# QZ1-boy/FCVSR

Hardware: AMD Instinct MI355X
Metric: SR frames/sec (7-frame window, 4x 180x320->720x1280) + PSNR vs ref (higher is better)
Workload: dtype bf16

## Files before the change

fcvsr_amd/engine.py:

```python
from __future__ import annotations

import ctypes as C
import math
import weakref
from collections import OrderedDict
from typing import Dict, List, Optional, Tuple

import numpy as np
import torch

from . import hip
from .hip import ACT_LEAKY, ACT_NONE, ACT_PRELU, ACT_RELU, check, lib, ptr, stream_ptr, view


_MASKS: Dict[Tuple[int, int, int], torch.Tensor] = {}


def band_masks_half(Q: int, H: int, W: int) -> torch.Tensor:
    key = (Q, H, W)
    if key not in _MASKS:
        n = 1024
        step = math.sqrt((n / 2) ** 2 + (n / 2) ** 2) / Q
        d2 = (np.arange(-(n // 2), n - n // 2, 1) ** 2).astype(np.float64)
        r2 = np.power(np.sqrt(d2[:, None] + d2[None, :]), 2)
# ... 140 lines not shown
    def _mask(self, Q, H, W, dev):
        key = (Q, H, W, str(dev))
        if key not in self._dev_masks:
            self._dev_masks[key] = band_masks_half(Q, H, W).to(dev)
        return self._dev_masks[key]

    def _conv(self, name, srcs, dst, *, stride=1, act=ACT_NONE, slope=0.0, slope_t=None, res=(), res_scale=(),
              ps=False, freq=False, direct=False, force_f16=False, rows=None, cols=None):
        self._convg(name, [dict(srcs=srcs, dst=dst, res=res, ps=ps)], stride=stride, act=act, slope=slope,
                    slope_t=slope_t, res_scale=res_scale, ps=ps, freq=freq, direct=direct, force_f16=force_f16, rows=rows,
                    cols=cols)
        return dst

    def _convg(self, name, groups, *, stride=1, act=ACT_NONE, slope=0.0, slope_t=None, res_scale=(), ps=False,
               freq=False, direct=False, force_f16=False, gc_wmask=None, rows=None, cols=None):
        ksz = self._par[name + ".weight"].shape[-1]
        any16 = any(t.dtype != torch.float32 for g in groups for t in list(g["srcs"]) + [g["dst"]])
        elig = self.precision != "f32" and not direct and hip.mfma_eligible(ksz, stride, groups)
        if any16 and not elig:
            raise RuntimeError(f"{name}: 16-bit activations require the MFMA path (ineligible shape/alignment)")
        if elig:
            dt = torch.bfloat16 if (self.precision == "bf16" or freq) else torch.float16
            if force_f16:
                dt = torch.float16
            w, b, cout, _ = self._weights(name, dt, ps, rows, cols)
            hip.conv2d_mfma(groups, w, ksz, cout, hip.BF16 if dt == torch.bfloat16 else hip.F16, stride=stride, bias=b, act=act,
                            slope=slope, slope_t=slope_t, res_scale=res_scale, pixel_shuffle=ps, gc_wmask=gc_wmask,
                            name=name)
            return True
        w, b, cout, _ = self._weights(name, "direct", False, rows, cols)
        wm = bm = None
        if (ksz in (1, 3) and stride == 1 and not direct and all(len(g["srcs"]) == 1 and g["srcs"][0].shape[3] % 32 == 0
                                                                  for g in groups) and (not ps or cout % 16 == 0)):
            wm, bm = self._weights(name, "f32mfma", ps, rows, cols)[:2]
        for g in groups:
            hip.conv2d(g["srcs"], w, ksz, cout, g["dst"], bias=b, stride=stride, act=act, slope=slope, slope_t=slope_t,
                       res=g.get("res", ()), res_scale=res_scale, pixel_shuffle=ps, name=name, w_f32mfma=wm, bias_f32mfma=bm)
        return False

    def _tap(self, name, t_nhwc):
        if self.taps is not None:
            self.taps[name] = t_nhwc.float().permute(0, 3, 1, 2).contiguous().clone()

    @staticmethod
    def _new(dev, *shape, dtype=torch.float32):
        return torch.empty(*shape, device=dev, dtype=dtype)

    def _channel_sum(self, t):
        B, H, W, Cc = t.shape
        nblk = (H * W + 255) // 256
        out = self._new(t.device, B, Cc)
        scratch = self._new(t.device, B * nblk * Cc)
        v = view(t)
        check(lib().fcvsr_channel_sum(C.byref(v), B, H, W, out.data_ptr(), scratch.data_ptr(), scratch.numel(),
                                      stream_ptr()), "fcvsr_channel_sum")
        return out

    def _ca_gate(self, sums, inv_hw, prefix, Bn, c):
        par = self._par
        w1, w2 = par[prefix + ".conv_du.0.weight"], par[prefix + ".conv_du.2.weight"]
        gate = self._new(sums.device, Bn, c)
        check(lib().fcvsr_ca_gate(sums.data_ptr(), inv_hw, w1.data_ptr(), w2.data_ptr(), Bn, c, w1.shape[0],
                                  gate.data_ptr(), stream_ptr()), "fcvsr_ca_gate")
        return gate

    def _mgaa(self, x1, x2, x3, tag):
        m = self._model()
        n, A = m.n_feats, m.ACNum
        dev = x1.device
        B, H, W, _ = x1.shape
        Wf = W // 2 + 1
        L = lib()
        st = stream_ptr()
        par = self._par

        spec = self._new(dev, 3, B, H, Wf, 2 * n)
        fs = 2 * n
        for i, xi in enumerate((x1, x2, x3)):
            v = view(xi)
            check(L.fcvsr_rfft2(C.byref(v), B, H, W, n, spec[i].data_ptr(), fs, 0, n, st), "fcvsr_rfft2")
        x1f, x2f, x3f = spec[0], spec[1], spec[2]

        fdt = self._adt(freq=True)
        off = self._new(dev, 2 * B, H, Wf, 2 * n, dtype=fdt)
        fused = fdt != torch.float32 and n == 64
        if fused:
            ws = [self._weights(f"MGAA.convfuse.{i}", torch.bfloat16)[0] for i in (0, 2, 4)]
            P2 = C.c_void_p * 2
            check(L.fcvsr_freq_mlp3(P2(x1f.data_ptr(), x3f.data_ptr()), P2(x2f.data_ptr(), x2f.data_ptr()), 2, fs,
                                    B * H * Wf, ws[0].data_ptr(), ws[1].data_ptr(), ws[2].data_ptr(),
                                    P2(off[:B].data_ptr(), off[B:].data_ptr()), 2 * n, st), "fcvsr_freq_mlp3")
        else:
            t0 = self._new(dev, 2 * B, H, Wf, 2 * n, dtype=fdt)
            t1 = self._new(dev, 2 * B, H, Wf, 2 * n, dtype=fdt)
            dirs = list(enumerate((x1f, x3f)))
            self._convg("MGAA.convfuse.0", [dict(srcs=[xa, x2f], dst=t0[d * B:(d + 1) * B]) for d, xa in dirs],
                        act=ACT_RELU, freq=True)
            self._convg("MGAA.convfuse.2", [dict(srcs=[t0], dst=t1)], act=ACT_RELU, freq=True)
            self._convg("MGAA.convfuse.4", [dict(srcs=[t1[d * B:(d + 1) * B]], dst=off[d * B:(d + 1) * B], res=[xa, x2f])
                                            for d, xa in dirs], res_scale=[1.0, -1.0], freq=True)
        sim = self._new(dev, B, H, Wf, 4)
        off4 = self._new(dev, 2 * B, H, Wf, 4)
        if fused:
            check(L.fcvsr_freq_head(x2f.data_ptr(), hip.F32, fs, B * H * Wf,
                                    self._weights("MGAA.convcrt.0", torch.bfloat16)[0].data_ptr(), None,
                                    self._weights("MGAA.convcrt.2", torch.bfloat16)[0].data_ptr(), sim.data_ptr(), st),
                  "fcvsr_freq_head(convcrt)")
        else:
            s0 = self._new(dev, B, H, Wf, n, dtype=fdt)
            self._conv("MGAA.convcrt.0", [x2f], s0, act=ACT_RELU, freq=True)
            self._conv("MGAA.convcrt.2", [s0], sim, freq=True)

        if fdt == torch.float32:
            c0 = self._new(dev, 2 * B, H, Wf, n, dtype=fdt)
            c1 = self._new(dev, 2 * B, H, Wf, n, dtype=fdt)
            corr = self._new(dev, B, H, Wf, 84)
            cv = view(corr)
            check(L.fcvsr_corr_lookup(x1f.data_ptr(), x2f.data_ptr(), fs, B, H, Wf, 2 * n, 4, Wf, C.byref(cv), st),
                  "fcvsr_corr_lookup")
            for d in range(2):
                self._conv("MGAA.convcorr.0", [off[d * B:(d + 1) * B], corr], c0[d * B:(d + 1) * B], act=ACT_RELU, freq=True)
            self._conv("MGAA.convcorr.2", [c0], c1, act=ACT_RELU, freq=True)
            self._conv("MGAA.convcorr.4", [c1], off4, freq=True)
        else:
            if fused:
                check(L.fcvsr_freq_head(off.data_ptr(), hip.BF16, 2 * n, 2 * B * H * Wf,
                                        self._weights("MGAA.convcorr.0", torch.bfloat16, cols=(0, 2 * n))[0].data_ptr(),
                                        self._weights("MGAA.convcorr.2", torch.bfloat16)[0].data_ptr(),
                                        self._weights("MGAA.convcorr.4", torch.bfloat16)[0].data_ptr(), off4.data_ptr(), st),
                      "fcvsr_freq_head(convcorr)")
            else:
                c0 = self._new(dev, 2 * B, H, Wf, n, dtype=fdt)
                c1 = self._new(dev, 2 * B, H, Wf, n, dtype=fdt)
                self._conv("MGAA.convcorr.0", [off], c0, act=ACT_RELU, freq=True, cols=(0, 2 * n))
            xs = min(Wf, 8)
            corr = self._new(dev, B, H, xs, 84)
            cv = view(corr)
            check(L.fcvsr_corr_lookup(x1f.data_ptr(), x2f.data_ptr(), fs, B, H, Wf, 2 * n, 4, xs, C.byref(cv), st),
                  "fcvsr_corr_lookup")
            off_s = off[:, :, :xs].to(torch.float32, memory_format=torch.contiguous_format)
            c0_s = self._new(dev, 2 * B, H, xs, n, dtype=fdt)
            for d in range(2):
                self._conv("MGAA.convcorr.0", [off_s[d * B:(d + 1) * B], corr], c0_s[d * B:(d + 1) * B], act=ACT_RELU,
                           freq=True)
            if fused:
                c1_s = self._new(dev, 2 * B, H, xs, n, dtype=fdt)
                off4_s = self._new(dev, 2 * B, H, xs, 4)
                self._conv("MGAA.convcorr.2", [c0_s], c1_s, act=ACT_RELU, freq=True)
                self._conv("MGAA.convcorr.4", [c1_s], off4_s, freq=True)
                off4[:, :, :xs].copy_(off4_s)
            else:
                c0[:, :, :xs].copy_(c0_s)
                self._conv("MGAA.convcorr.2", [c0], c1, act=ACT_RELU, freq=True)
                self._conv("MGAA.convcorr.4", [c1], off4, freq=True)

        ospec = self._new(dev, B, H, Wf, 8 * A)
        u = self._new(dev, 2 * B, H, Wf, 4)
        ntile = ((H + 15) // 16) * ((Wf + 15) // 16)
        partial = self._new(dev, 2 * B * ntile * 4)
        for i in range(A):
            pre = f"MGAA.MConvB.{i}"
            w1 = self._weights(pre + ".conv1", "direct")[0]
            w2 = self._weights(pre + ".conv2", "direct")[0]
            check(L.fcvsr_convblk(off4.data_ptr(), w1.data_ptr(), w2.data_ptr(), par[pre + ".relu.weight"].data_ptr(),
                                  par[pre + ".conv1.weight"].shape[-1], par[pre + ".CA.conv_du.0.weight"].data_ptr(),
                                  par[pre + ".CA.conv_du.2.weight"].data_ptr(), sim.data_ptr(), B, 2, H, Wf, u.data_ptr(),
                                  partial.data_ptr(), partial.numel(), ospec.data_ptr(), 8 * A, 0, 4 * A, A, i, st),
                  "fcvsr_convblk")
        offsets = self._new(dev, B, H, W, 4 * A)
        ov = view(offsets)
        check(L.fcvsr_irfft2(ospec.data_ptr(), 8 * A, 4 * A, 0, B, H, W, 4 * A, None, None, C.byref(ov), st),
              "fcvsr_irfft2")

        kp = self._new(dev, B, H, W, n, dtype=self._adt())
        k0 = self._new(dev, B, H, W, n, dtype=self._adt())
        fused_iac = n % 32 == 0
        self._conv("MGAA.conv_KP", [x2], kp)
        self._conv("MGAA.F.0", [kp], k0)
        fold_f1 = fused_iac and n == 64 and self.precision != "f32" and self._model().fold_f1
        if not fold_f1:
            K = self._new(dev, B, H, W, A * 3 * n, dtype=self._adt() if fused_iac else torch.float32)
            self._conv("MGAA.F.1", [k0], K)

        fdt_act = x1.dtype
        al = self._new(dev, B, H, W, 2 * n, dtype=fdt_act)
        ping = [self._new(dev, B, H, W, n, dtype=fdt_act), self._new(dev, B, H, W, n, dtype=fdt_act)]
        if not fused_iac:
            if fdt_act != torch.float32:
                raise RuntimeError("16-bit activations need the fused IAC kernel (n_features % 32 == 0)")
            s = self._new(dev, B, H, W, n)
            vbuf = self._new(dev, B, H, W, n)
        if fused_iac and n % 64 == 0:
            ping2 = [self._new(dev, B, H, W, n, dtype=fdt_act), self._new(dev, B, H, W, n, dtype=fdt_act)]
            V2 = hip.View * 2
            cur = [x1, x3]
            fins = V2(view(x1), view(x3))
            if fold_f1:
                wk, bk, _, _ = self._weights("MGAA.F.1", self._adt())
                k0_v = view(k0)
            for i in range(A):
                if not fold_f1:
                    k_v = view(K[..., i * 3 * n:(i + 1) * 3 * n])
                if i == A - 1:
                    dsts = [al[..., :n], al[..., n:]]
                else:
                    dsts = [ping[i % 2], ping2[i % 2]]
                prevs = V2(view(cur[0]), view(cur[1]))
                offs = V2(view(offsets[..., 2 * i:2 * i + 2]), view(offsets[..., 2 * (A + i):2 * (A + i) + 2]))
                dv2 = V2(view(dsts[0]), view(dsts[1]))
                if fold_f1:
                    check(L.fcvsr_iac_step2_fused(prevs, offs, C.byref(k0_v), wk.data_ptr() + i * 3 * n * 64 * 2,
                                                  bk.data_ptr() + i * 3 * n * 4, fins, 0.1, B, H, W, dv2, st),
                          "fcvsr_iac_step2_fused")
                else:
                    check(L.fcvsr_iac_step2(prevs, offs, C.byref(k_v), fins, 0.1, B, H, W, dv2, st), "fcvsr_iac_step2")
                cur = dsts
        else:
            for d, fin in enumerate((x1, x3)):
                cur = fin
                fv = view(fin)
                for i in range(A):
                    g = d * A + i
                    o_v = view(offsets[..., 2 * g:2 * g + 2])
# ... 381 lines not shown
```

fcvsr_amd/hip.py:

```python
from __future__ import annotations

import ctypes as C
import os
from typing import Optional, Sequence

import torch

_HERE = os.path.dirname(os.path.abspath(__file__))
LIB_PATH = os.path.join(_HERE, "lib", "libfcvsr_hip.so")

F32, BF16, F16 = 0, 1, 2
ACT_NONE, ACT_RELU, ACT_LEAKY, ACT_PRELU = 0, 1, 2, 3
_DT = {torch.float32: F32, torch.bfloat16: BF16, torch.float16: F16}


class View(C.Structure):
    _fields_ = [("ptr", C.c_void_p), ("sb", C.c_int64), ("sy", C.c_int64), ("sx", C.c_int64), ("sc", C.c_int64),
                ("c", C.c_int32), ("dtype", C.c_int32)]


class GcFinishLevel(C.Structure):
    _fields_ = [("partial", C.c_void_p), ("add", C.c_void_p), ("nparts", C.c_int32)]


class GcPartialLevel(C.Structure):
    _fields_ = [("r", C.c_void_p), ("partial", C.c_void_p), ("B", C.c_int32), ("H", C.c_int32), ("W", C.c_int32)]


class GcApplyLevel(C.Structure):
    _fields_ = [("r", C.c_void_p), ("add", C.c_void_p), ("z", C.c_void_p), ("out", C.c_void_p), ("pool", C.c_void_p),
                ("B", C.c_int32), ("H", C.c_int32), ("W", C.c_int32)]


class XscaleLevel(C.Structure):
    _fields_ = [("x", C.c_void_p), ("r", C.c_void_p), ("dn", C.c_void_p), ("up", C.c_void_p), ("out", C.c_void_p),
                ("r_scale", C.c_float), ("dn_pooled", C.c_int32), ("B", C.c_int32), ("H", C.c_int32), ("W", C.c_int32)]


class RcbTailArgs(C.Structure):
    _fields_ = [("x", C.c_void_p * 3), ("r", C.c_void_p * 3), ("z", C.c_void_p * 3), ("add", C.c_void_p * 3),
                ("out", C.c_void_p * 3), ("r1", C.c_void_p), ("u1", C.c_void_p), ("u2", C.c_void_p), ("w_up", C.c_void_p),
                ("b_up", C.c_void_p), ("w_dn", C.c_void_p), ("b_dn", C.c_void_p), ("B", C.c_int32), ("H", C.c_int32),
                ("W", C.c_int32)]


class ConvDesc(C.Structure):
    _fields_ = [("n_src", C.c_int32), ("src", View * 3), ("B", C.c_int32), ("H", C.c_int32), ("W", C.c_int32),
                ("kh", C.c_int32), ("kw", C.c_int32), ("stride", C.c_int32), ("pad", C.c_int32),
                ("cout", C.c_int32), ("weight", C.c_void_p), ("cout_pad", C.c_int32), ("bias", C.c_void_p),
                ("act", C.c_int32), ("slope", C.c_float), ("slope_ptr", C.c_void_p), ("n_res", C.c_int32),
                ("res", View * 2), ("res_scale", C.c_float * 2), ("dst", View), ("pixel_shuffle", C.c_int32),
                ("gc_wmask", C.c_void_p), ("gc_partial", C.c_void_p)]


PROFILE = None
COMPUTE_DTYPE = "f32"
DOMINANT_KERNEL = "conv_direct_kernel"


class HipError(RuntimeError):
    pass


_lib: Optional[C.CDLL] = None

_VP, _I, _I64, _F = C.c_void_p, C.c_int, C.c_int64, C.c_float
_PV = C.POINTER(View)
SIGNATURES = {
    "fcvsr_last_error": [],
    "fcvsr_last_conv_kernel": [],
    "fcvsr_conv2d_wgrad_scratch_elems": [C.c_int] * 7,
    "fcvsr_conv2d_wgrad": [C.c_void_p, C.c_void_p, C.c_int, C.c_int, C.c_int, C.c_int, C.c_int, C.c_int, C.c_int, C.c_void_p, C.c_void_p,
                           C.c_longlong, C.c_int, C.c_void_p],
    "fcvsr_conv2d_wgrad_mfma_eligible": [C.c_int] * 6,
    "fcvsr_conv2d_wgrad_mfma_scratch_elems": [C.c_int] * 7,
    "fcvsr_conv2d_wgrad_mfma": [C.c_void_p, C.c_void_p, C.c_int, C.c_int, C.c_int, C.c_int, C.c_int, C.c_int, C.c_int, C.c_void_p, C.c_void_p,
                                C.c_void_p, C.c_longlong, C.c_int, C.c_int, C.c_void_p],
    "fcvsr_abi_version": [],
    "fcvsr_device_count": [],
    "fcvsr_conv2d": [C.POINTER(ConvDesc), _VP],
    "fcvsr_conv2d_f32mfma": [C.POINTER(ConvDesc), _VP],
    "fcvsr_conv2d_f32mfma_eligible": [C.POINTER(ConvDesc)],
    "fcvsr_conv2d_mfma": [C.POINTER(ConvDesc), _I, _I, _VP],
    "fcvsr_rfft2": [_PV, _I, _I, _I, _I, _VP, _I64, _I, _I, _VP],
    "fcvsr_irfft2": [_VP, _I64, _I, _I, _I, _I, _I, _I, _VP, _VP, _PV, _VP],
    "fcvsr_irfft2_bands": [_VP, _I64, _I, _I, _I, _I, _I, _I, _VP, _I, _VP, _PV, _VP],
    "fcvsr_corr_lookup": [_VP, _VP, _I64, _I, _I, _I, _I, _I, _I, _PV, _VP],
    "fcvsr_channel_sum": [_PV, _I, _I, _I, _VP, _VP, _I64, _VP],
    "fcvsr_ca_gate": [_VP, _F, _VP, _VP, _I, _I, _I, _VP, _VP],
    "fcvsr_convblk_tail": [_VP, _VP, _VP, _I, _I, _I, _I, _VP, _I64, _I, _I, _I, _I, _VP],
    "fcvsr_convblk": [_VP, _VP, _VP, _VP, _I, _VP, _VP, _VP, _I, _I, _I, _I, _VP, _VP, _I64, _VP, _I64, _I, _I, _I, _I, _VP],
    "fcvsr_warp": [_PV, _PV, _I, _I, _I, _PV, _VP],
    "fcvsr_sac_v": [_PV, _PV, _I, _I, _I, _PV, _VP],
    "fcvsr_sac_h": [_PV, _PV, _PV, _F, _I, _I, _I, _PV, _VP],
    "fcvsr_iac_step": [_PV, _PV, _PV, _PV, _F, _I, _I, _I, _PV, _VP],
    "fcvsr_feat_extract": [_PV, _I, _I, _I, _VP, _VP, _I, _VP, _VP, _VP, _I, _VP],
    "fcvsr_freq_head": [_VP, _I, _I64, _I64, _VP, _VP, _VP, _VP, _VP],
    "fcvsr_freq_mlp3": [_VP, _VP, _I, _I64, _I64, _VP, _VP, _VP, _VP, _I64, _VP],
    "fcvsr_iac_step2": [_PV, _PV, _PV, _PV, _F, _I, _I, _I, _PV, _VP],
    "fcvsr_iac_step2_fused": [_PV, _PV, _PV, _VP, _VP, _PV, _F, _I, _I, _I, _PV, _VP],
    "fcvsr_divenh": [_I, _I, _VP, _VP, _VP, _VP, _VP, _VP, _F, _VP, _VP, _VP, _VP, _I64, _I, _I, _I, _I, _VP],
    "fcvsr_divenh_apply_next": [_I, _VP, _VP, _VP, _VP, _VP, _VP, _F, _VP, _VP, _VP, _VP, _VP, _VP, _VP, _I64, _I, _I, _I, _I, _VP],
    "fcvsr_scale_add": [_VP, _VP, _VP, _I, _VP, _I, _I, _I, _I, _I, _VP],
    "fcvsr_gc_context": [_VP, _VP, _VP, _VP, _I, _I, _I, _I, _VP, _VP, _I64, _VP],
    "fcvsr_gc_finish": [_VP, _I, _VP, _VP, _I, _I, _VP, _VP],
    "fcvsr_gc_apply": [_VP, _VP, _VP, _VP, _I, _F, _I, _I, _I, _I, _VP],
    "fcvsr_xscale": [_VP, _VP, _F, _VP, _VP, _VP, _I, _I, _I, _I, _I, _VP],
    "fcvsr_gc_finish_levels": [C.POINTER(GcFinishLevel), _I, _VP, _VP, _I, _I, _VP],
    "fcvsr_gc_partial_levels": [C.POINTER(GcPartialLevel), _I, _I, _VP, _I, _VP],
    "fcvsr_gc_apply_levels": [C.POINTER(GcApplyLevel), _I, _I, _I, _F, _I, _VP],
    "fcvsr_xscale_levels": [C.POINTER(XscaleLevel), _I, _I, _I, _VP],
    "fcvsr_rcb_level0": [_VP, _VP, _VP, _VP, _VP, _VP, _VP, _F, _F, _I, _I, _I, _I, _I, _VP],
    "fcvsr_rcb_tail": [C.POINTER(RcbTailArgs), _F, _I, _I, _VP],
    "fcvsr_pixel_shuffle": [_VP, _VP, _I, _I, _I, _I, _VP],
    "fcvsr_bilinear_up4": [_PV, _I, _I, _I, _PV, _VP],
    "fcvsr_tail_fused": [_PV, _VP, _VP, _VP, _VP, _VP, _I, _I, _I, _PV, _VP],
    "fcvsr_conv_last": [_PV, _VP, _VP, _I, _I, _I, _I, _PV, _VP],
    "fcvsr_pack_weight_mfma": [_VP, _I, _I, _I, _I, _VP, _I, _I, _I, _I, _VP],
    "fcvsr_pack_weights_multi_block_elems": [],
    "fcvsr_pack_weights_mfma_multi": [_VP, _I, _I, _I, _VP],
    "fcvsr_act_bwd": [_VP, _VP, _VP, _F, C.c_longlong, _VP],
    "fcvsr_colsum_scratch_elems": [C.c_longlong, _I],
    "fcvsr_colsum": [_VP, C.c_longlong, _I, _VP, _VP, C.c_longlong, _I, _VP],
    "fcvsr_iac_bwd_sac": [_VP, _VP, _VP, _VP, _PV, _F, _I, _I, _I, _I, _VP, _I, _VP, _PV, _I, _VP],
    "fcvsr_iac_bwd_warp": [_VP, _PV, _VP, _PV, _I, _I, _I, _I, _VP, _VP, _VP],
    "fcvsr_prelu_fwd": [_VP, _VP, _VP, C.c_longlong, _VP],
    "fcvsr_prelu_bwd": [_VP, _VP, _VP, _VP, _VP, _VP, C.c_longlong, _VP],
    "fcvsr_wgrad_cout1_scratch_elems": [_I, _I, _I],
    "fcvsr_wgrad_cout1": [_VP, _VP, _I, _I, _I, _I, _VP, _VP, C.c_longlong, _I, _VP],
    "fcvsr_conv2d_wgrad_mfma_groups_scratch_elems": [_VP, _VP, _VP, _I, _I, _I, _I, _I],
    "fcvsr_conv2d_wgrad_mfma_groups": [_VP, _VP, _VP, _VP, _VP, _I, _I, _I, _I, _VP, _VP, _VP, C.c_longlong, _I, _I, _VP],
    "fcvsr_up2_adjoint": [_VP, _VP, _I, _I, _I, _I, _VP],
    "fcvsr_pool2_adjoint": [_VP, _VP, _I, _I, _I, _I, _VP],
    "fcvsr_rcbt_nblk": [_I],
    "fcvsr_rcbt_stat_elems": [],
    "fcvsr_rcbt_forward": [_VP, _VP, _VP, _VP, _VP, _F, _I, _I, _I, _VP, _VP, _VP, C.c_longlong, _VP],
    "fcvsr_rcbt_backward": [_VP, _VP, _VP, _VP, _VP, _VP, _F, _I, _I, _I, _VP, _VP, _VP, _VP, _VP, C.c_longlong, _I, _VP],
    "fcvsr_divenh_band_nblk": [_I],
    "fcvsr_divenh_band_stat_elems": [_I],
    "fcvsr_divenh_band_forward": [_VP, _VP, _VP, _VP, _VP, _VP, _VP, _I, _I, _I, _VP, _VP, _VP, _VP, C.c_longlong, _VP],
    "fcvsr_divenh_band_backward": [_VP, _VP, _VP, _VP, _VP, _VP, _VP, _VP, _VP, _VP, _I, _I, _I, _VP, _VP, _VP, _VP, _VP, _VP, _VP, _VP,
                                   C.c_longlong, _I, _VP],
    "fcvsr_corr_lookup_bwd": [_VP, _VP, _I64, _I, _I, _I, _I, _I, _I, _PV, _VP, _VP, _VP],
    "fcvsr_frame_metrics_scratch_bytes": [_I] * 6,
    "fcvsr_frame_metrics": [_VP, C.POINTER(C.c_int64), _I, _VP, C.POINTER(C.c_int64), _I, _I, _I, _I, _I, _I,
                            C.POINTER(C.c_double), _VP, _VP, C.c_longlong, _VP],
}
_RESTYPES = {"fcvsr_last_error": C.c_char_p, "fcvsr_last_conv_kernel": C.c_char_p, "fcvsr_conv2d_wgrad_scratch_elems": C.c_longlong,
             "fcvsr_conv2d_wgrad_mfma_scratch_elems": C.c_longlong, "fcvsr_colsum_scratch_elems": C.c_longlong,
             "fcvsr_wgrad_cout1_scratch_elems": C.c_longlong, "fcvsr_conv2d_wgrad_mfma_groups_scratch_elems": C.c_longlong,
             "fcvsr_frame_metrics_scratch_bytes": C.c_longlong}


def lib() -> C.CDLL:
    global _lib
    if _lib is None:
        if not os.path.exists(LIB_PATH):
            raise HipError(f"{LIB_PATH} not found: run `python -m fcvsr_amd.build` (hipcc, gfx950). "
                           "fcvsr_amd has no CPU fallback.")
        l = C.CDLL(LIB_PATH)
        for name, args in SIGNATURES.items():
            fn = getattr(l, name, None)
            if fn is None:
                continue
            fn.argtypes = args
            fn.restype = _RESTYPES.get(name, C.c_int)
        _lib = l
    return _lib


def check(rc: int, what: str) -> None:
    if rc != 0:
        msg = lib().fcvsr_last_error()
        raise HipError(f"{what} failed (rc={rc}): {msg.decode() if msg else ''}")


def stream_ptr() -> int:
    return torch.cuda.current_stream().cuda_stream


def view(t: torch.Tensor) -> View:
# ... 164 lines not shown
```

include/fcvsr_hip.h:

```cpp
#ifndef FCVSR_HIP_H
#define FCVSR_HIP_H

#include <stdint.h>

#ifdef __cplusplus
extern "C" {
#endif

#define FCVSR_ABI_VERSION 2

enum { FCVSR_E_ARG = -1, FCVSR_E_UNSUPPORTED = -2, FCVSR_E_NOGPU = -3 };
enum { FCVSR_F32 = 0, FCVSR_BF16 = 1, FCVSR_F16 = 2 };
enum { FCVSR_ACT_NONE = 0, FCVSR_ACT_RELU = 1, FCVSR_ACT_LEAKY = 2, FCVSR_ACT_PRELU = 3 };

typedef struct fcvsr_view {
  void*   ptr;
  int64_t sb, sy, sx, sc;
  int32_t c;
  int32_t dtype;
} fcvsr_view;

typedef struct fcvsr_conv_desc {
  int32_t     n_src;
  fcvsr_view  src[3];
// ... 37 lines not shown
                           int transposed, void* stream);
int fcvsr_pack_weights_multi_block_elems(void);
int fcvsr_pack_weights_mfma_multi(const long long* tab, int n_items, int total_blocks, int dtype, void* stream);
int fcvsr_act_bwd(const float* g, const float* y, float* out, float slope, long long n, void* stream);
long long fcvsr_colsum_scratch_elems(long long npix, int C);
int fcvsr_colsum(const float* x, long long npix, int C, float* out, float* scratch, long long scratch_elems, int accumulate, void* stream);
int fcvsr_rcbt_nblk(int HW);
int fcvsr_rcbt_stat_elems(void);
int fcvsr_rcbt_forward(const float* r, const float* z, const float* wmask, const float* w1, const float* w2, float slope, int B, int HW,
                       int C, float* out, float* stats, float* scratch, long long scratch_elems, void* stream);
int fcvsr_rcbt_backward(const float* r, const float* g, const float* wmask, const float* w1, const float* w2, const float* stats,
                        float slope, int B, int HW, int C, float* gr, float* dwmask, float* dw1, float* dw2, float* scratch,
                        long long scratch_elems, int accumulate , void* stream);

int fcvsr_divenh_band_nblk(int HW);
int fcvsr_divenh_band_stat_elems(int C);
int fcvsr_divenh_band_forward(const float* f, const float* sf, const float* so, const float* a, const float* b, const float* w1,
                              const float* w2, int B, int HW, int C, float* sf_out, float* so_out, float* stats, float* scratch,
                              long long scratch_elems, void* stream);
int fcvsr_divenh_band_backward(const float* f, const float* sf, const float* so, const float* a, const float* b, const float* w1,
                               const float* w2, const float* stats, const float* gsf, const float* gso, int B, int HW, int C, float* gf,
                               float* gsf_out, float* gso_out, float* ga, float* gb, float* dw1, float* dw2, float* scratch,
                               long long scratch_elems, int accumulate, void* stream);
int fcvsr_corr_lookup_bwd(const float* x1f, const float* x2f, int64_t pix_stride, int B, int H, int Wf, int C, int radius, int x_count,
                          const fcvsr_view* g, float* gx1_zeroed, float* gx2_zeroed, void* stream);
int fcvsr_prelu_fwd(const float* x, const float* slope, float* y, long long n, void* stream);
int fcvsr_prelu_bwd(const float* g, const float* x, const float* slope, float* gx, float* gslope, float* scratch, long long n, void* stream);
long long fcvsr_wgrad_cout1_scratch_elems(int B, int H, int C);
int fcvsr_wgrad_cout1(const float* x, const float* gy, int B, int H, int W, int C, float* dw, float* scratch, long long scratch_elems,
                      int accumulate, void* stream);
int fcvsr_iac_bwd_sac(const float* gy, const float* yout, const float* v, const float* s, const fcvsr_view* k1, float slope, int B, int H,
                      int W, int C, float* gfin, int fin_accumulate, float* gv, const fcvsr_view* gk, int k_accumulate, void* stream);
int fcvsr_iac_bwd_warp(const float* gv, const fcvsr_view* k1, const float* prev, const fcvsr_view* off, int B, int H, int W, int C,
                       float* gprev_zeroed, float* goff, void* stream);
long long fcvsr_conv2d_wgrad_mfma_groups_scratch_elems(const int* B, const int* H, const int* W, int n_groups, int cin, int cout, int kh,
                                                       int kw);
int fcvsr_conv2d_wgrad_mfma_groups(const fcvsr_view* xs, const fcvsr_view* gys, const int* B, const int* H, const int* W, int n_groups, int kh,
                                   int kw, int pad, float* dw, float* dbias, float* scratch, long long scratch_elems, int dw_accumulate,
                                   int dbias_accumulate, void* stream);
int fcvsr_up2_adjoint(const float* g, float* out, int B, int H, int W, int C, void* stream);
int fcvsr_pool2_adjoint(const float* g, float* out, int B, int H, int W, int C, void* stream);
int fcvsr_rfft2(const fcvsr_view* src, int B, int H, int W, int n,
                float* spec, int64_t pix_stride, int im_off, int re_off, void* stream);
int fcvsr_irfft2(const float* spec, int64_t pix_stride, int im_off, int re_off, int B, int H, int W, int n,
                 const float* mask, float* work, const fcvsr_view* dst, void* stream);
int fcvsr_irfft2_bands(const float* spec, int64_t pix_stride, int im_off, int re_off, int B, int H, int W, int n,
                       const float* masks, int n_bands, float* work, const fcvsr_view* dst, void* stream);

int fcvsr_feat_extract(const fcvsr_view* x, int B, int H, int W, const void* w, const float* bias, int n_blk,
                       void* const* dst, const int64_t* dst_pix_stride, const int32_t* dst_ch_off, int dst_dtype,
                       void* stream);

int fcvsr_corr_lookup(const float* x1f, const float* x2f, int64_t pix_stride, int B, int H, int Wf, int C, int radius,
                      int x_count, const fcvsr_view* dst, void* stream);
int fcvsr_channel_sum(const fcvsr_view* src, int B, int H, int W, float* out, float* scratch, int64_t scratch_elems,
                      void* stream);
int fcvsr_ca_gate(const float* sum, float inv_hw, const float* w1, const float* w2, int B, int c, int cr,
                  float* gate, void* stream);
int fcvsr_convblk_tail(const float* u, const float* gate, const float* sim, int B, int ndir, int H, int Wf,
                       float* spec, int64_t pix_stride, int re_off, int im_off, int g_stride, int g0, void* stream);
int fcvsr_convblk(const float* x, const float* w1, const float* w2, const float* prelu_slope, int ksize, const float* ca_w1,
                  const float* ca_w2, const float* sim, int B, int ndir, int H, int Wf, float* u_scratch,
                  float* partial_scratch, int64_t partial_elems, float* spec, int64_t pix_stride, int re_off, int im_off,
                  int g_stride, int g0, void* stream);
int fcvsr_warp(const fcvsr_view* src, const fcvsr_view* off, int B, int H, int W, const fcvsr_view* dst, void* stream);
int fcvsr_sac_v(const fcvsr_view* s, const fcvsr_view* k1, int B, int H, int W, const fcvsr_view* dst, void* stream);
int fcvsr_sac_h(const fcvsr_view* v, const fcvsr_view* k1, const fcvsr_view* feat_in, float slope,
                int B, int H, int W, const fcvsr_view* dst, void* stream);

int fcvsr_iac_step(const fcvsr_view* prev, const fcvsr_view* off, const fcvsr_view* k1, const fcvsr_view* feat_in,
                   float slope, int B, int H, int W, const fcvsr_view* dst, void* stream);
int fcvsr_iac_step2(const fcvsr_view* prev, const fcvsr_view* off, const fcvsr_view* k1, const fcvsr_view* feat_in,
                    float slope, int B, int H, int W, const fcvsr_view* dst, void* stream);
int fcvsr_iac_step2_fused(const fcvsr_view* prev, const fcvsr_view* off, const fcvsr_view* k0, const void* wk,
                          const float* kbias, const fcvsr_view* feat_in, float slope, int B, int H, int W,
                          const fcvsr_view* dst, void* stream);

int fcvsr_freq_mlp3(const float* const* xa, const float* const* xb, int n_dirs, int64_t src_pix_stride, int64_t npix,
                    const void* w0, const void* w2, const void* w4, void* const* dst, int64_t dst_pix_stride, void* stream);

int fcvsr_freq_head(const void* x, int x_dtype, int64_t x_pix_stride, int64_t npix, const void* w0, const void* w_mid,
                    const void* w_last, float* out, void* stream);

int fcvsr_divenh(int mode, int first, const float* f, float* s_f, float* s_o, const float* a, const float* b,
                 const float* mean_f_sum, float inv_hw, const float* g1, const float* g2,
                 float* sums, float* scratch, int64_t scratch_elems, int B, int H, int W, int C, void* stream);
int fcvsr_divenh_apply_next(int first, const float* f, float* s_f, float* s_o, const float* a, const float* b,
                            const float* mean_f_sum, float inv_hw, const float* g1, const float* g2,
                            const float* f_next, const float* a_next, const float* b_next, float* sums,
                            float* scratch, int64_t scratch_elems, int B, int H, int W, int C, void* stream);
int fcvsr_scale_add(const float* z, const float* gate, const void* x, int x_dtype, void* out, int out_dtype, int B, int H,
                    int W, int C, void* stream);

int fcvsr_gc_context(const float* r, const float* wmask, const float* w1, const float* w2, int B, int H, int W, int C,
                     float* add, float* scratch, int64_t scratch_elems, void* stream);
int fcvsr_gc_finish(const float* partial, int nparts, const float* w1, const float* w2, int B, int C, float* add,
                    void* stream);
int fcvsr_gc_apply(const float* r, const float* add, const void* z, void* out, int io_dtype, float slope,
                   int B, int H, int W, int C, void* stream);
int fcvsr_xscale(const void* x, const void* r, float r_scale, const void* dn, const void* up, void* out, int io_dtype,
                 int B, int H, int W, int C, void* stream);

typedef struct {
  const float* partial;
  float*       add;
  int32_t      nparts;
} fcvsr_gc_finish_level;
int fcvsr_gc_finish_levels(const fcvsr_gc_finish_level* lv, int n_levels, const float* w1, const float* w2, int B, int C,
                           void* stream);
typedef struct {
  const void*  r;
  const float* add;
  const void*  z;
  void*        out;
  void*        pool;
  int32_t      B, H, W;
} fcvsr_gc_apply_level;
int fcvsr_gc_apply_levels(const fcvsr_gc_apply_level* lv, int n_levels, int io_dtype, int r_dtype, float slope, int C,
                          void* stream);
typedef struct {
  const void* x;
  const void* r;
  const void* dn;
  const void* up;
  void*       out;
  float       r_scale;
  int32_t     dn_pooled;
  int32_t     B, H, W;
} fcvsr_xscale_level;
int fcvsr_xscale_levels(const fcvsr_xscale_level* lv, int n_levels, int io_dtype, int C, void* stream);

int fcvsr_rcb_level0(const void* x, const void* r, const float* add, const void* z, const void* up, void* out, void* pool,
                     float slope, float r_scale, int io_dtype, int B, int H, int W, int C, void* stream);

typedef struct {
  const void*  x[3];
  const void*  r[3];
  const void*  z[3];
  const float* add[3];
  void*        out[3];
  void*        r1;
  void*        u1;
  void*        u2;
  const void*  w_up;
  const float* b_up;
  const void*  w_dn;
  const float* b_dn;
  int32_t      B, H, W;
} fcvsr_rcb_tail_args;
int fcvsr_rcb_tail(const fcvsr_rcb_tail_args* a, float slope, int io_dtype, int C, void* stream);

typedef struct {
  const void* r;
  float*      partial;
  int32_t     B, H, W;
} fcvsr_gc_partial_level;
int fcvsr_gc_partial_levels(const fcvsr_gc_partial_level* lv, int n_levels, int r_dtype, const float* wmask, int C, void* stream);

int fcvsr_pixel_shuffle(const float* src, float* dst, int B, int H, int W, int C, void* stream);
int fcvsr_bilinear_up4(const fcvsr_view* src, int B, int H, int W, const fcvsr_view* dst, void* stream);

int fcvsr_tail_fused(const fcvsr_view* u1, const void* w2, const float* b2, const float* slope, const void* wl,
                     const float* bl, int B, int H2, int W2, const fcvsr_view* out, void* stream);
int fcvsr_conv_last(const fcvsr_view* u, const void* w, const float* bias, int B, int H, int W, int C, const fcvsr_view* out, void* stream);

enum { FCVSR_QUANT_NONE = 0, FCVSR_QUANT_TRUNCATE = 1, FCVSR_QUANT_ROUND = 2 };
// ... 10 lines not shown
```

Before: 867.3.

## Fuse MGAA frequency-domain MLPs into one MFMA kernel

Replaces the separate freq_mlp3 (convfuse) and two freq_head launches (convcrt, convcorr) with a single kernel that runs all three MLP chains per 128-pixel tile, keeping hidden activations in LDS. It writes off4 and sim directly, plus only the small strip of offsets needed by the correlation path, so the full bf16 offset tensor is never written to or reread from global memory. The cost is a complex unit schedule with high register and LDS use and fewer launches that can overlap, which may limit occupancy.

Result: no change. 874.0 (median of 6 runs) (+0.8%).

```diff
diff --git a/fcvsr_amd/csrc/freq_front.hip b/fcvsr_amd/csrc/freq_front.hip
--- /dev/null
+++ b/fcvsr_amd/csrc/freq_front.hip
@@ -0,0 +1,253 @@
+#include "common.h"
+#include "mfma_util.h"
+#include <utility>
+
+namespace fcvsr {
+
+constexpr int kFfC = 128;
+constexpr int kFfPix = 128;
+constexpr int kFfLD = 64 + 8;
+constexpr int kFfTD = kFfC + 8;
+constexpr int kFfTBytes = kFfPix * kFfTD * 2;
+constexpr int kFfBBytes = kFfC * kFfLD * 2;
+constexpr int kFfLds = kFfTBytes + kFfBBytes;
+
+struct FreqFrontArgs {
+  const float* x[3];
+  long long sx;
+  int npix, Wf, strip_w, n_rows;
+  const uint16_t* w[8];
+  float* off4;
+  float* sim;
+  float* strip;
+};
+
+enum { kSrcT = 0, kSrcXa = 1, kSrcX2 = 2 };
+__host__ __device__ constexpr int ff_local(int k) { return k < 12 ? k : (k < 15 ? k - 12 + 100 : k - 15); }
+__host__ __device__ constexpr int ff_src(int k) {
+  return ff_local(k) >= 100 ? (ff_local(k) == 102 ? kSrcT : kSrcX2)
+                            : (ff_local(k) < 2 ? kSrcXa : (ff_local(k) < 4 ? kSrcX2 : kSrcT));
+}
+__host__ __device__ constexpr int ff_pc0(int k) {
+  return ff_local(k) >= 100 ? (ff_local(k) - 100) * 64 % 128 : (ff_local(k) & 1) * 64 * (ff_local(k) < 10);
+}
+__host__ __device__ constexpr int ff_wid(int k) {
+  return ff_local(k) >= 100 ? (ff_local(k) == 102 ? 7 : 6)
+                            : (ff_local(k) < 4 ? 0 : ff_local(k) < 6 ? 1 : ff_local(k) < 8 ? 2 : ff_local(k) < 10 ? 3
+                                                                                                    : ff_local(k) - 6);
+}
+__host__ __device__ constexpr int ff_wc0(int k) {
+  return ff_local(k) >= 100 ? (ff_local(k) == 101 ? 64 : 0)
+                            : (ff_local(k) < 4 ? ff_local(k) * 64 : ff_local(k) < 10 ? (ff_local(k) & 1) * 64 : 0);
+}
+__host__ __device__ constexpr int ff_ntile(int k) {
+  return ff_local(k) >= 100 ? (ff_local(k) == 102 ? 1 : 2) : (ff_local(k) < 8 ? 4 : ff_local(k) < 11 ? 2 : 1);
+}
+__host__ __device__ constexpr int ff_cin(int k) {
+  return ff_wid(k) == 0 ? 256 : (ff_wid(k) <= 3 || ff_wid(k) == 6) ? 128 : 64;
+}
+
+template <class F, int... K>
+__device__ __forceinline__ void ff_units(F& f, std::integer_sequence<int, K...>) {
+  (f(std::integral_constant<int, K>{}), ...);
+}
+
+__global__ __launch_bounds__(256, 3) void freq_front_kernel(FreqFrontArgs a) {
+  extern __shared__ __align__(16) unsigned char lds[];
+  uint16_t* T_s = reinterpret_cast<uint16_t*>(lds);
+  uint16_t* A_s = T_s;
+  uint16_t* B_s = reinterpret_cast<uint16_t*>(lds + kFfTBytes);
+  const int tid = threadIdx.x;
+  const int lane = tid & 63, wave = tid >> 6;
+  const int r = lane & 31, h = lane >> 5;
+  const int flat0 = blockIdx.x * kFfPix;
+  const int npix = a.npix;
+
+  f32x16_t acc[4];
+  auto zero_acc = [&]() __attribute__((always_inline)) {
+#pragma unroll
+    for (int nf = 0; nf < 4; ++nf)
+#pragma unroll
+      for (int i = 0; i < 16; ++i) acc[nf][i] = 0.f;
+  };
+  auto mma_chunk = [&](const uint16_t* prow, int ntile) __attribute__((always_inline)) {
+    const uint16_t* wrow = B_s + r * kFfLD + h * 8;
+#pragma unroll
+    for (int kk = 0; kk < 4; ++kk) {
+      const uint4 pf = *reinterpret_cast<const uint4*>(prow + kk * 16);
+      uint4 wf[4];
+#pragma unroll
+      for (int nf = 0; nf < 4; ++nf)
+        if (nf < ntile) wf[nf] = *reinterpret_cast<const uint4*>(wrow + nf * 32 * kFfLD + kk * 16);
+#pragma unroll
+      for (int nf = 0; nf < 4; ++nf)
+        if (nf < ntile) acc[nf] = mfma<true>(wf[nf], pf, acc[nf]);
+      if (kk & 1) __builtin_amdgcn_sched_barrier(0);
+    }
+  };
+  auto store_hidden = [&](int ntile) __attribute__((always_inline)) {
+    uint16_t* trow = T_s + (wave * 32 + r) * kFfTD;
+#pragma unroll
+    for (int nf = 0; nf < 4; ++nf)
+#pragma unroll
+      for (int g = 0; g < 4; ++g)
+        if (nf < ntile) {
+          const float4 v = make_float4(fmaxf(acc[nf][4 * g], 0.f), fmaxf(acc[nf][4 * g + 1], 0.f), fmaxf(acc[nf][4 * g + 2], 0.f),
+                                       fmaxf(acc[nf][4 * g + 3], 0.f));
+          *reinterpret_cast<uint2*>(trow + nf * 32 + 8 * g + 4 * h) = cvt4<true>(v);
+        }
+  };
+
+  auto rsrc = [](const void* p, unsigned bytes) __attribute__((always_inline)) {
+    return __builtin_amdgcn_make_buffer_rsrc(const_cast<void*>(p), (short)0, (int)bytes, 0x00020000);
+  };
+  const unsigned xbytes = (unsigned)a.npix * (unsigned)a.sx * 4u;
+  const __amdgpu_buffer_rsrc_t xr[3] = {rsrc(a.x[0], xbytes), rsrc(a.x[1], xbytes), rsrc(a.x[2], xbytes)};
+  auto bld = [](__amdgpu_buffer_rsrc_t rs, unsigned off) __attribute__((always_inline)) {
+    return __builtin_amdgcn_raw_buffer_load_b128(rs, off, 0, 0);
+  };
+  auto gld4 = [&](int src, unsigned off) __attribute__((always_inline)) { return __builtin_bit_cast(float4, bld(xr[src], off)); };
+  const unsigned sxb = (unsigned)a.sx * 4u;
+  const int q = tid & 15, p0 = tid >> 4;
+  float4 xv[8];
+  uint4 wv[4];
+  auto load_x = [&](int src, int c0) __attribute__((always_inline)) {
+#pragma unroll
+    for (int i = 0; i < 8; ++i) {
+      xv[i] = gld4(src, (unsigned)(flat0 + p0 + i * 16) * sxb + c0 * 4 + q * 16);
+    }
+  };
+  auto put_x = [&]() __attribute__((always_inline)) {
+#pragma unroll
+    for (int i = 0; i < 8; ++i) *reinterpret_cast<uint2*>(A_s + (p0 + i * 16) * kFfLD + q * 4) = cvt4<true>(xv[i]);
+  };
+  auto load_w = [&](int k) __attribute__((always_inline)) {
+    const __amdgpu_buffer_rsrc_t wr = rsrc(a.w[ff_wid(k)], (unsigned)(32 * ff_ntile(k) * ff_cin(k) * 2));
+#pragma unroll
+    for (int u = 0; u < 4; ++u)
+      if (u < ff_ntile(k)) wv[u] = __builtin_bit_cast(uint4, bld(wr, (unsigned)(((tid >> 3) + 32 * u) * ff_cin(k) + ff_wc0(k) + (tid & 7) * 8) * 2u));
+  };
+  auto put_w = [&](int ntile) __attribute__((always_inline)) {
+#pragma unroll
+    for (int u = 0; u < 4; ++u)
+      if (u < ntile) *reinterpret_cast<uint4*>(B_s + ((tid >> 3) + 32 * u) * kFfLD + (tid & 7) * 8) = wv[u];
+  };
+  auto issue = [&](int k) __attribute__((always_inline)) {
+    if (ff_src(k) == kSrcXa) load_x(k < 12 ? 0 : 2, ff_pc0(k));
+    else if (ff_src(k) == kSrcX2) load_x(1, ff_pc0(k));
+    load_w(k);
+  };
+
+  const int pix_w = flat0 + wave * 32 + r;
+  auto epilogue = [&](int d) __attribute__((always_inline)) {
+    const unsigned pofs = (unsigned)pix_w * sxb;
+    int srow = -1;
+    if (pix_w < npix) {
+      const int row = pix_w / a.Wf, x = pix_w - row * a.Wf;
+      if (x < a.strip_w) srow = (d * a.n_rows + row) * a.strip_w + x;
+    }
+    uint16_t* trow = T_s + (wave * 32 + r) * kFfTD;
+#pragma unroll
+    for (int half = 0; half < 2; ++half) {
+      __builtin_amdgcn_sched_barrier(0);
+      float4 ra[2][4], rb[2][4];
+#pragma unroll
+      for (int nf2 = 0; nf2 < 2; ++nf2)
+#pragma unroll
+        for (int g = 0; g < 4; ++g) {
+          const unsigned off = pofs + ((half * 2 + nf2) * 32 + 8 * g + 4 * h) * 4u;
+          ra[nf2][g] = gld4(d ? 2 : 0, off);
+          rb[nf2][g] = gld4(1, off);
+        }
+#pragma unroll
+      for (int nf2 = 0; nf2 < 2; ++nf2)
+#pragma unroll
+        for (int g = 0; g < 4; ++g) {
+          const int nf = half * 2 + nf2;
+          const float4 av = ra[nf2][g], bv = rb[nf2][g];
+          const float4 v = make_float4(fmaf(-1.f, bv.x, fmaf(1.f, av.x, acc[nf][4 * g])),
+                                       fmaf(-1.f, bv.y, fmaf(1.f, av.y, acc[nf][4 * g + 1])),
+                                       fmaf(-1.f, bv.z, fmaf(1.f, av.z, acc[nf][4 * g + 2])),
+                                       fmaf(-1.f, bv.w, fmaf(1.f, av.w, acc[nf][4 * g + 3])));
+          const uint2 o = cvt4<true>(v);
+          *reinterpret_cast<uint2*>(trow + nf * 32 + 8 * g + 4 * h) = o;
+          if (srow >= 0) {
+            float f[4];
+            cvt16x4_to_f32<true>(o, f);
+            *reinterpret_cast<float4*>(a.strip + (long long)srow * kFfC + nf * 32 + 8 * g + 4 * h) = make_float4(f[0], f[1], f[2], f[3]);
+          }
+        }
+    }
+  };
+  auto store_out4 = [&](float* out) __attribute__((always_inline)) {
+    if (h == 0 && pix_w < npix)
+      *reinterpret_cast<float4*>(out + (long long)pix_w * 4) = make_float4(acc[0][0], acc[0][1], acc[0][2], acc[0][3]);
+  };
+
+  auto unit = [&](auto kc) __attribute__((always_inline)) {
+    constexpr int k = decltype(kc)::value;
+    constexpr int l = ff_local(k);
+    if (l == 0 || l == 4 || l == 6 || l == 8 || l == 10 || l == 11 || l == 100 || l == 102) zero_acc();
+    __syncthreads();
+    if (ff_src(k) != kSrcT) put_x();
+    put_w(ff_ntile(k));
+    if (k + 1 < 27) issue(k + 1);
+    __syncthreads();
+    const uint16_t* prow = ff_src(k) != kSrcT ? A_s + (wave * 32 + r) * kFfLD + h * 8
+                                              : T_s + (wave * 32 + r) * kFfTD + ff_pc0(k) + h * 8;
+    mma_chunk(prow, ff_ntile(k));
+    if (l == 3 || l == 101) {
+      __syncthreads();
+      store_hidden(ff_ntile(k));
+    } else if (l == 5 || l == 9 || l == 10) {
+      __builtin_amdgcn_wave_barrier();
+      store_hidden(ff_ntile(k));
+    } else if (l == 7) {
+      __builtin_amdgcn_wave_barrier();
+      epilogue(k < 12 ? 0 : 1);
+    } else if (l == 11) {
+      store_out4(a.off4 + (k < 12 ? 0 : (long long)npix * 4));
+    } else if (l == 102) {
+      store_out4(a.sim);
+    }
+  };
+  issue(0);
+  ff_units(unit, std::make_integer_sequence<int, 27>{});
+}
+
+}
+
+using namespace fcvsr;
+
+extern "C" int fcvsr_freq_front(const float* x1f, const float* x2f, const float* x3f, int64_t src_pix_stride, int64_t npix,
+                                int Wf, const void* fuse_w0, const void* fuse_w2, const void* fuse_w4, const void* corr_w0,
+                                const void* corr_w2, const void* corr_w4, const void* crt_w0, const void* crt_w2, float* off4,
+                                float* sim, float* strip, int strip_w, void* stream) {
+  const void* w[8] = {fuse_w0, fuse_w2, fuse_w4, corr_w0, corr_w2, corr_w4, crt_w0, crt_w2};
+  FCVSR_CHECK_ARG(x1f && x2f && x3f && off4 && sim && strip, "null argument");
+  for (int i = 0; i < 8; ++i) FCVSR_CHECK_ARG(w[i] && ((uintptr_t)w[i] % 16) == 0, "weights: non-null, 16-byte aligned");
+  FCVSR_CHECK_ARG(((uintptr_t)x1f % 16) == 0 && ((uintptr_t)x2f % 16) == 0 && ((uintptr_t)x3f % 16) == 0 &&
+                      ((uintptr_t)off4 % 16) == 0 && ((uintptr_t)sim % 16) == 0 && ((uintptr_t)strip % 16) == 0,
+                  "spectra / outputs must be 16-byte aligned");
+  FCVSR_CHECK_ARG(npix > 0 && npix < (1ll << 30) && src_pix_stride >= kFfC && src_pix_stride % 4 == 0, "bad sizes / strides");
+  FCVSR_CHECK_ARG(Wf > 0 && npix % Wf == 0 && strip_w > 0 && strip_w <= Wf, "npix = rows * Wf, 0 < strip_w <= Wf");
+  FCVSR_CHECK_ARG((npix + kFfPix) * src_pix_stride * 4 < (1ll << 32), "tensor too large for 32-bit offsets");
+  FreqFrontArgs a;
+  a.x[0] = x1f; a.x[1] = x2f; a.x[2] = x3f;
+  a.sx = src_pix_stride; a.npix = (int)npix; a.Wf = Wf; a.strip_w = strip_w; a.n_rows = (int)(npix / Wf);
+  for (int i = 0; i < 8; ++i) a.w[i] = (const uint16_t*)w[i];
+  a.off4 = off4; a.sim = sim; a.strip = strip;
+  static DevOnce attr;
+  {
+    hipError_t e = once_per_device(attr, [&] {
+      return hipFuncSetAttribute((const void*)freq_front_kernel, hipFuncAttributeMaxDynamicSharedMemorySize, kFfLds);
+    });
+    if (e != hipSuccess) {
+      set_error("fcvsr_freq_front: %s", hipGetErrorString(e));
+      return (int)e;
+    }
+  }
+  hipLaunchKernelGGL(freq_front_kernel, dim3(cdiv(npix, kFfPix)), dim3(256), kFfLds, (hipStream_t)stream, a);
+  FCVSR_LAUNCH_CHECK();
+  return 0;
+}
diff --git a/fcvsr_amd/engine.py b/fcvsr_amd/engine.py
--- a/fcvsr_amd/engine.py
+++ b/fcvsr_amd/engine.py
@@ -246,15 +246,20 @@
         x1f, x2f, x3f = spec[0], spec[1], spec[2]
 
         fdt = self._adt(freq=True)
-        off = self._new(dev, 2 * B, H, Wf, 2 * n, dtype=fdt)
         fused = fdt != torch.float32 and n == 64
+        sim = self._new(dev, B, H, Wf, 4)
+        off4 = self._new(dev, 2 * B, H, Wf, 4)
         if fused:
-            ws = [self._weights(f"MGAA.convfuse.{i}", torch.bfloat16)[0] for i in (0, 2, 4)]
-            P2 = C.c_void_p * 2
-            check(L.fcvsr_freq_mlp3(P2(x1f.data_ptr(), x3f.data_ptr()), P2(x2f.data_ptr(), x2f.data_ptr()), 2, fs,
-                                    B * H * Wf, ws[0].data_ptr(), ws[1].data_ptr(), ws[2].data_ptr(),
-                                    P2(off[:B].data_ptr(), off[B:].data_ptr()), 2 * n, st), "fcvsr_freq_mlp3")
+            xs = min(Wf, 8)
+            off_s = self._new(dev, 2 * B, H, xs, 2 * n)
+            wb = lambda name, **kw: self._weights(name, torch.bfloat16, **kw)[0].data_ptr()
+            check(L.fcvsr_freq_front(x1f.data_ptr(), x2f.data_ptr(), x3f.data_ptr(), fs, B * H * Wf, Wf,
+                                     wb("MGAA.convfuse.0"), wb("MGAA.convfuse.2"), wb("MGAA.convfuse.4"),
+                                     wb("MGAA.convcorr.0", cols=(0, 2 * n)), wb("MGAA.convcorr.2"), wb("MGAA.convcorr.4"),
+                                     wb("MGAA.convcrt.0"), wb("MGAA.convcrt.2"), off4.data_ptr(), sim.data_ptr(),
+                                     off_s.data_ptr(), xs, st), "fcvsr_freq_front")
         else:
+            off = self._new(dev, 2 * B, H, Wf, 2 * n, dtype=fdt)
             t0 = self._new(dev, 2 * B, H, Wf, 2 * n, dtype=fdt)
             t1 = self._new(dev, 2 * B, H, Wf, 2 * n, dtype=fdt)
             dirs = list(enumerate((x1f, x3f)))
@@ -263,14 +268,6 @@
             self._convg("MGAA.convfuse.2", [dict(srcs=[t0], dst=t1)], act=ACT_RELU, freq=True)
             self._convg("MGAA.convfuse.4", [dict(srcs=[t1[d * B:(d + 1) * B]], dst=off[d * B:(d + 1) * B], res=[xa, x2f])
                                             for d, xa in dirs], res_scale=[1.0, -1.0], freq=True)
-        sim = self._new(dev, B, H, Wf, 4)
-        off4 = self._new(dev, 2 * B, H, Wf, 4)
-        if fused:
-            check(L.fcvsr_freq_head(x2f.data_ptr(), hip.F32, fs, B * H * Wf,
-                                    self._weights("MGAA.convcrt.0", torch.bfloat16)[0].data_ptr(), None,
-                                    self._weights("MGAA.convcrt.2", torch.bfloat16)[0].data_ptr(), sim.data_ptr(), st),
-                  "fcvsr_freq_head(convcrt)")
-        else:
             s0 = self._new(dev, B, H, Wf, n, dtype=fdt)
             self._conv("MGAA.convcrt.0", [x2f], s0, act=ACT_RELU, freq=True)
             self._conv("MGAA.convcrt.2", [s0], sim, freq=True)
@@ -287,22 +284,16 @@
             self._conv("MGAA.convcorr.2", [c0], c1, act=ACT_RELU, freq=True)
             self._conv("MGAA.convcorr.4", [c1], off4, freq=True)
         else:
-            if fused:
-                check(L.fcvsr_freq_head(off.data_ptr(), hip.BF16, 2 * n, 2 * B * H * Wf,
-                                        self._weights("MGAA.convcorr.0", torch.bfloat16, cols=(0, 2 * n))[0].data_ptr(),
-                                        self._weights("MGAA.convcorr.2", torch.bfloat16)[0].data_ptr(),
-                                        self._weights("MGAA.convcorr.4", torch.bfloat16)[0].data_ptr(), off4.data_ptr(), st),
-                      "fcvsr_freq_head(convcorr)")
-            else:
+            if not fused:
                 c0 = self._new(dev, 2 * B, H, Wf, n, dtype=fdt)
                 c1 = self._new(dev, 2 * B, H, Wf, n, dtype=fdt)
                 self._conv("MGAA.convcorr.0", [off], c0, act=ACT_RELU, freq=True, cols=(0, 2 * n))
-            xs = min(Wf, 8)
+                xs = min(Wf, 8)
+                off_s = off[:, :, :xs].to(torch.float32, memory_format=torch.contiguous_format)
             corr = self._new(dev, B, H, xs, 84)
             cv = view(corr)
             check(L.fcvsr_corr_lookup(x1f.data_ptr(), x2f.data_ptr(), fs, B, H, Wf, 2 * n, 4, xs, C.byref(cv), st),
                   "fcvsr_corr_lookup")
-            off_s = off[:, :, :xs].to(torch.float32, memory_format=torch.contiguous_format)
             c0_s = self._new(dev, 2 * B, H, xs, n, dtype=fdt)
             for d in range(2):
                 self._conv("MGAA.convcorr.0", [off_s[d * B:(d + 1) * B], corr], c0_s[d * B:(d + 1) * B], act=ACT_RELU,
diff --git a/fcvsr_amd/hip.py b/fcvsr_amd/hip.py
--- a/fcvsr_amd/hip.py
+++ b/fcvsr_amd/hip.py
@@ -97,6 +97,7 @@
     "fcvsr_feat_extract": [_PV, _I, _I, _I, _VP, _VP, _I, _VP, _VP, _VP, _I, _VP],
     "fcvsr_freq_head": [_VP, _I, _I64, _I64, _VP, _VP, _VP, _VP, _VP],
     "fcvsr_freq_mlp3": [_VP, _VP, _I, _I64, _I64, _VP, _VP, _VP, _VP, _I64, _VP],
+    "fcvsr_freq_front": [_VP, _VP, _VP, _I64, _I64, _I] + [_VP] * 11 + [_I, _VP],
     "fcvsr_iac_step2": [_PV, _PV, _PV, _PV, _F, _I, _I, _I, _PV, _VP],
     "fcvsr_iac_step2_fused": [_PV, _PV, _PV, _VP, _VP, _PV, _F, _I, _I, _I, _PV, _VP],
     "fcvsr_divenh": [_I, _I, _VP, _VP, _VP, _VP, _VP, _VP, _F, _VP, _VP, _VP, _VP, _I64, _I, _I, _I, _I, _VP],
diff --git a/include/fcvsr_hip.h b/include/fcvsr_hip.h
--- a/include/fcvsr_hip.h
+++ b/include/fcvsr_hip.h
@@ -143,6 +143,11 @@
 int fcvsr_freq_head(const void* x, int x_dtype, int64_t x_pix_stride, int64_t npix, const void* w0, const void* w_mid,
                     const void* w_last, float* out, void* stream);
 
+int fcvsr_freq_front(const float* x1f, const float* x2f, const float* x3f, int64_t src_pix_stride, int64_t npix, int Wf,
+                     const void* fuse_w0, const void* fuse_w2, const void* fuse_w4, const void* corr_w0, const void* corr_w2,
+                     const void* corr_w4, const void* crt_w0, const void* crt_w2, float* off4, float* sim, float* strip,
+                     int strip_w, void* stream);
+
 int fcvsr_divenh(int mode, int first, const float* f, float* s_f, float* s_o, const float* a, const float* b,
                  const float* mean_f_sum, float inv_hw, const float* g1, const float* g2,
                  float* sums, float* scratch, int64_t scratch_elems, int B, int H, int W, int C, void* stream);
```
